# mmbajo/PROBA-V

Hardware: AMD Instinct MI355X
Metric: LR-patches/sec fwd+bwd (WDSR-B r12 t9, 16x16, bs128) (higher is better)
Workload: dtype f32 (products as 3 scaled-fp16-piece MFMA products, f32 accumulate)

## Files before the change

include/probav_hip.h:

```cpp
#ifndef PROBAV_HIP_H
#define PROBAV_HIP_H
#include <stddef.h>
#include <stdint.h>
#ifdef __cplusplus
extern "C" {
#endif

#define PROBAV_ABI_VERSION 7

typedef struct probav_net_cfg {
    int32_t scale;
    int32_t num_filters;
    int32_t num_res_blocks;
    int32_t exp_rate;
    int32_t dec_channels;
    int32_t num_img_lr;
    int32_t patch_size_lr;
    int32_t max_shift;
    float mean, std;
    int32_t in_channels;
} probav_net_cfg;

typedef struct probav_engine probav_engine;

// ... 67 lines not shown
int probav_clip_round(const float* in, float* out, size_t n, float lo, float hi, void* stream);

int probav_conv3d_forward(const int32_t geom[17], const float* x, const float* gate, const float* w,
                          const float* bias, const float* skip, float* y, int impl, void* stream);
size_t probav_conv3d_wgrad_scratch_bytes(const int32_t geom[17], int impl);
int probav_conv3d_wgrad(const int32_t geom[17], const float* x, const float* dy, const float* gate,
                        float* dw, float* db, void* scratch, size_t scratch_bytes, int impl, void* stream);
int probav_pw_forward(const float* x, const float* w1, const float* b1, const float* w2, const float* b2, float* dec,
                      int64_t nvox, int64_t vox_per_sample, int D, int impl, void* stream);
size_t probav_pw_backward_scratch_bytes(int D);
int probav_pw_backward(const float* x, const float* d_dec, const float* d_skip, const float* w1, const float* b1,
                       const float* w2, float* dx, float* dw1, float* db1, float* dw2, float* db2, void* scratch,
                       size_t scratch_bytes, int64_t nvox, int64_t vox_per_sample, int D, int impl, void* stream);
int probav_input_grad(int batch, int H, int T, int C, const float* g, const float* act0, const float* wmain, const float* d1,
                      const float* gate1 , const float* w1, float stdv, float* dx, void* stream);
int64_t probav_weff_count(const probav_engine* e);
int64_t probav_cout_total(const probav_engine* e);
int probav_wn_forward(probav_engine* e, const float* params, float* weff, float* weffT, float* inv_norm, void* stream);
int probav_wn_backward(probav_engine* e, const float* params, const float* dweff, const float* inv_norm,
                       float* grads, void* stream);

int probav_engine_side_stream(probav_engine* e, int mode);

int probav_mfma_probe(const void* seed, float* sink, int iters, int launches, void* stream);
int probav_mfma_probe_shape(const void* seed, float* sink, int iters, int launches, int shape, void* stream);

#define PROBAV_VIEW_ACT 0
#define PROBAV_VIEW_DEC 1
#define PROBAV_VIEW_RED 2
#define PROBAV_VIEW_RESID1 3
#define PROBAV_VIEW_INPUT 4
int probav_workspace_view(const probav_engine* e, int batch, int training, int kind, int index, int64_t* offset_floats, int64_t* count);
int probav_debug_hidden(probav_engine* e, const float* params, const void* ws , size_t ws_bytes, int batch, int block, float* hidden,
                        float* dec_scratch ,
                        const void* wcache , void* stream);
int probav_debug_hidden_from_forward_kernel(int on);

#define PROBAV_PLAN_NONE 0
#define PROBAV_PLAN_CW4 1
#define PROBAV_PLAN_PP 2
#define PROBAV_PLAN_PSTRIP 3
#define PROBAV_PLAN_STRIP 4
#define PROBAV_PLAN_ROWTILE 5
#define PROBAV_PLAN_DIRECT 6
#define PROBAV_PLAN_WG4 7
#define PROBAV_PLAN_WGRAD_X6 8
// ... 103 lines not shown
```

proba-v_amd/_lib.py:

```python
import ctypes
import os
from ctypes import POINTER, c_char, c_char_p, c_float, c_int, c_int32, c_int64, c_size_t, c_uint8, c_void_p

CSRC = os.path.join(os.path.dirname(os.path.abspath(__file__)), "csrc")
LIB_PATH = os.path.join(CSRC, "libprobav_hip.so")

PROBAV_OK, PROBAV_EINVAL, PROBAV_ENOSPACE, PROBAV_EHIP = 0, -1, -2, -3


class NetCfg(ctypes.Structure):
    _fields_ = [("scale", c_int32), ("num_filters", c_int32), ("num_res_blocks", c_int32), ("exp_rate", c_int32),
                ("dec_channels", c_int32), ("num_img_lr", c_int32), ("patch_size_lr", c_int32),
                ("max_shift", c_int32), ("mean", c_float), ("std", c_float), ("in_channels", c_int32)]


class GuardCtl(ctypes.Structure):
    _fields_ = [("scale", c_float), ("skip", ctypes.c_uint32), ("skipped_total", ctypes.c_uint32), ("norm", c_float)]


SIGNATURES = {
    "probav_abi_version": (c_int, []),
    "probav_last_error": (c_char_p, []),
    "probav_engine_create": (c_int, [POINTER(NetCfg), POINTER(c_void_p)]),
    "probav_engine_destroy": (None, [c_void_p]),
# ... 20 lines not shown
    "probav_clip_round": (c_int, [c_void_p, c_void_p, c_size_t, c_float, c_float, c_void_p]),
    "probav_nadam_step": (c_int, [c_void_p, c_void_p, c_void_p, c_void_p, c_int64, c_float, c_float, c_float, c_float,
                                  c_float, c_float, c_float, c_void_p]),
    "probav_grad_guard_scratch_bytes": (c_size_t, [c_int64]),
    "probav_grad_guard": (c_int, [c_void_p, c_int64, c_float, c_int, c_void_p, c_size_t, c_void_p, c_void_p]),
    "probav_nadam_step_guarded": (c_int, [c_void_p, c_void_p, c_void_p, c_void_p, c_void_p, c_int64, c_float, c_float, c_float, c_float,
                                          c_float, c_float, c_float, c_float, c_void_p, c_void_p]),
    "probav_optimizer_step_fused_guarded": (c_int, [c_void_p, c_void_p, c_void_p, c_void_p, c_void_p, c_float, c_float, c_float, c_float, c_float, c_float,
                                                    c_float, c_void_p, c_size_t, c_void_p, c_float, c_void_p, c_void_p]),
    "probav_conv3d_forward": (c_int, [POINTER(c_int32 * 17), c_void_p, c_void_p, c_void_p, c_void_p, c_void_p,
                                      c_void_p, c_int, c_void_p]),
    "probav_conv3d_wgrad_scratch_bytes": (c_size_t, [POINTER(c_int32 * 17), c_int]),
    "probav_conv3d_wgrad": (c_int, [POINTER(c_int32 * 17), c_void_p, c_void_p, c_void_p, c_void_p, c_void_p,
                                    c_void_p, c_size_t, c_int, c_void_p]),
    "probav_pw_forward": (c_int, [c_void_p, c_void_p, c_void_p, c_void_p, c_void_p, c_void_p, c_int64, c_int64, c_int, c_int, c_void_p]),
    "probav_pw_backward_scratch_bytes": (c_size_t, [c_int]),
    "probav_pw_backward": (c_int, [c_void_p] * 12 + [c_size_t, c_int64, c_int64, c_int, c_int, c_void_p]),
    "probav_weff_count": (c_int64, [c_void_p]),
    "probav_cout_total": (c_int64, [c_void_p]),
    "probav_wn_forward": (c_int, [c_void_p, c_void_p, c_void_p, c_void_p, c_void_p, c_void_p]),
    "probav_wn_backward": (c_int, [c_void_p, c_void_p, c_void_p, c_void_p, c_void_p, c_void_p]),
    "probav_workspace_view": (c_int, [c_void_p, c_int, c_int, c_int, c_int, POINTER(c_int64), POINTER(c_int64)]),
    "probav_engine_side_stream": (c_int, [c_void_p, c_int]),
    "probav_weight_cache_build": (c_int, [c_void_p, c_void_p, c_void_p, c_size_t, c_void_p]),
    "probav_mfma_probe": (c_int, [c_void_p, c_void_p, c_int, c_int, c_void_p]),
    "probav_mfma_probe_shape": (c_int, [c_void_p, c_void_p, c_int, c_int, c_int, c_void_p]),
    "probav_debug_hidden": (c_int, [c_void_p, c_void_p, c_void_p, c_size_t, c_int, c_int, c_void_p, c_void_p, c_void_p, c_void_p]),
    "probav_debug_hidden_from_forward_kernel": (c_int, [c_int]),
    "probav_plan_conv": (c_int, [POINTER(c_int32 * 17), c_int, c_int, c_int, c_int, POINTER(c_int32 * 8)]),
    "probav_plan_pw": (c_int, [c_int64, c_int64, c_int, c_int, c_int, POINTER(c_int32 * 8)]),
    "probav_engine_set_gemm_route": (c_int, [c_void_p, c_int]),
    "probav_engine_gemm_route": (c_int, [c_void_p]),
    "probav_gemm_conv3d_forward": (c_int, [POINTER(c_int32 * 17), c_void_p, c_void_p, c_void_p, c_void_p, c_void_p, c_void_p, c_void_p]),
    "probav_gemm_conv3d_wgrad_scratch_bytes": (c_size_t, [POINTER(c_int32 * 17)]),
    "probav_gemm_conv3d_wgrad": (c_int, [POINTER(c_int32 * 17), c_void_p, c_void_p, c_void_p, c_void_p, c_void_p, c_void_p, c_size_t, c_void_p]),
    "probav_plan_conv_gemm": (c_int, [POINTER(c_int32 * 17), c_int, c_int, c_int, c_int, POINTER(c_int32 * 8)]),
    "probav_engine_route_counts": (c_int, [c_void_p, c_int, POINTER(c_int32 * 4)]),
    "probav_engine_launched_counts": (c_int, [c_void_p, POINTER(c_int32 * 4), c_int]),
    "probav_engine_set_gemm_pair": (c_int, [c_void_p, c_int]),
    "probav_engine_gemm_pair": (c_int, [c_void_p]),
    "probav_engine_pair_kind": (c_int, [c_void_p]),
    "probav_plan_pw_gemm": (c_int, [c_int, c_int, c_int, c_int64, c_int, POINTER(c_int32 * 8)]),
    "probav_engine_set_gemm_x6": (c_int, [c_void_p, c_int]),
    "probav_engine_gemm_x6": (c_int, [c_void_p]),
    "probav_engine_gemm_arith": (c_int, [c_void_p]),
    "probav_plan_conv_gemm_x6": (c_int, [POINTER(c_int32 * 17), c_int, c_int, c_int, POINTER(c_int32 * 8)]),
# ... 96 lines not shown
```

proba-v_amd/csrc/engine.hip:

```cpp
#include "probav_common.h"
#include "../../include/probav_hip.h"
#include <stdio.h>
#include <string.h>
#include <array>
#include <string>
#include <vector>

using namespace probav;

#include "kernels_mfma.h"
#include "kernels_x6.h"
#include "kernels_gemm.h"
#include "kernels_gemm_pw.h"
#include "kernels_gemm_x6.h"

struct ConvFrags { long f32 = -1, x6 = -1, h3 = -1, h3t = -1; };
struct PwFrags { long w1 = -1, w2 = -1, w2b = -1, w1c = -1; };

struct LayerRec {
    char name[32];
    WnLayer wn;
    int kh, kw, kt;
    ConvFrags pk[2];
};

enum class PairKind { none = 0, tuned = 1, gemm = 2 };
struct Family {
    bool mfma;
    bool strip;
    bool x6;
    int arith;
    PairKind pw_fused;
    bool gemm;
    int gemm_arith;
    bool gemm_exotic;
};
static Family make_family(int impl, bool pw_mfma, bool gemm = false, bool pair_gemm = false, bool gemm_x6 = false, bool gemm_exotic = false)
{
    Family f;
    f.mfma = impl >= 1; f.strip = impl >= 2; f.x6 = impl >= 3; f.arith = impl >= 4 ? 2 : (impl >= 3 ? 1 : 0);
    f.gemm = f.mfma && gemm;
    f.gemm_arith = f.gemm && gemm_x6 ? 1 : 0;
    f.gemm_exotic = f.gemm && gemm_exotic;
    f.pw_fused = !f.mfma ? PairKind::none : (pw_mfma ? PairKind::tuned : (f.gemm && pair_gemm ? PairKind::gemm : PairKind::none));
    return f;
}

struct probav_engine {
    probav_net_cfg cfg;
    std::vector<LayerRec> layers;
    int64_t nparams = 0, weff_count = 0, cout_total = 0, cin_total = 0;
    WnLayer* d_layers = nullptr;
    Family fam = {};
    int impl = 4;
    bool gemm = false;
    bool gemm_pair = false;
    bool gemm_x6 = false;
    bool gemm_exotic = false;
    bool pw_gemm = false;
    int32_t launched[4] = {0, 0, 0, 0};
    int iMain = -1, iResid1 = -1, iResid2 = -1, iResid3 = -1, iUp = -1;
    std::vector<int> iExp, iDec, iNorm, iRed;
    ReduceSide side = {};
    int side_mode = 2;
    bool side_tried = false;
    struct RedSpec { int k, p, pt, refl, refl_t; };
    std::vector<RedSpec> redSpec;
    int Hin = 0;
    std::vector<PackJob> jobs;
    PackJob* d_jobs = nullptr;
    int64_t wpack_count = 0;
    std::vector<std::array<PwFrags, 3>> pkBlk;
    bool pw_mfma = false;
    bool fwd_amax = false;
    PairKind fwd_pair = PairKind::none;
    int fwd_gemm_arith = 0;
    bool fwd_gemm_exotic = false;
    bool prof_on = false;
    unsigned prof_mask = ~0u;
    std::vector<hipEvent_t> prof_ev;
    std::vector<int> prof_cls;
    std::vector<double> prof_macs;
    size_t prof_used = 0;
};

static Family engine_family(const probav_engine* e) { return make_family(e->impl, e->pw_mfma, e->gemm, e->gemm_pair && e->pw_gemm, e->gemm_x6, e->gemm_exotic); }

enum { CLS_WN = 0, CLS_SMALL, CLS_CONV3_FWD, CLS_CONV3_BWD_DATA, CLS_CONV3_WGRAD, CLS_PW_FWD, CLS_PW_BWD_DATA, CLS_PW_WGRAD,
// ... 531 lines not shown
}
static int gemm_pair_backward_launch(const PassBufs& b, const Launch& L, const float* x, const float* dT, const float* dOut, float* dX, unsigned* ay, hipStream_t s)
{
    const probav_engine* e = b.e;
    const ConvGeom& g = L.g;
    const int i = L.i, D = e->cfg.dec_channels;
    if (L.kind != LaunchKind::fused || gemm_pw_backward_slab_floats(g.Cin, g.Cout, D, in_voxels(g)) > L.slab.floats) { set_error("probav_backward: the general fused pointwise pair's launch is not in the launch list, or its slab region is too small", hipSuccess); return PROBAV_EINVAL; }
    const WnLayer &we = e->layers[e->iExp[i]].wn, &wd = e->layers[e->iDec[i]].wn;
    CK(gemm_pw_backward(x, dT, dOut, b.dv.weff + we.w_off, b.params + we.b_off, b.dv.weff + wd.w_off, dX, b.dweff2 + we.w_off, b.dweff2 + wd.w_off,
                        b.grads + we.b_off, b.grads + wd.b_off, b.slabs + L.slab.off, in_voxels(g), g.Cin, g.Cout, D, s));
    if (ay) CK(amax_tensor(dX, (size_t)g.Hi * g.Wi * g.Ti * g.Cin, g.N, ay, s));
    return PROBAV_OK;
}

extern "C" {

int probav_abi_version(void) { return PROBAV_ABI_VERSION; }
int probav_engine_side_stream(probav_engine* e, int mode)
{
    if (!e || mode < 0 || mode > 2) { set_error("probav_engine_side_stream: bad argument", hipSuccess); return PROBAV_EINVAL; }
    e->side_mode = mode;
    return PROBAV_OK;
}
int probav_mfma_probe(const void* seed, float* sink, int iters, int launches, void* stream)
{
    if (!seed || !sink || iters < 1 || launches < 1) { set_error("probav_mfma_probe: null/invalid argument", hipSuccess); return PROBAV_EINVAL; }
    return mfma_probe(seed, sink, iters, launches, (hipStream_t)stream);
}
int probav_mfma_probe_shape(const void* seed, float* sink, int iters, int launches, int shape, void* stream)
{
    if (!seed || !sink || iters < 1 || launches < 1 || shape < 0 || shape > 1) { set_error("probav_mfma_probe_shape: null/invalid argument", hipSuccess); return PROBAV_EINVAL; }
    return mfma_probe(seed, sink, iters, launches, (hipStream_t)stream, shape);
}
const char* probav_last_error(void) { return probav::last_error(); }

int probav_engine_create(const probav_net_cfg* cfg, probav_engine** out)
{
    if (!cfg || !out) { set_error("probav_engine_create: null argument", hipSuccess); return PROBAV_EINVAL; }
    const int T = cfg->num_img_lr;
    if (cfg->scale != 3 || cfg->max_shift != 2 * cfg->scale) {
        set_error("probav_engine_create: the reference graph only closes for scale=3, maxShift=6 (models/modelsTF.py:45-53)", hipSuccess);
        return PROBAV_EINVAL;
    }
    if (T != 7 && T != 9 && T != 13 && T != 19) {
        set_error("probav_engine_create: numImgLR must be 7, 9, 13 or 19 (models/modelsTF.py:62-69)", hipSuccess);
        return PROBAV_EINVAL;
// ... 460 lines not shown
    CK(reduce_flush(s));
    for (int i = R - 1; i >= 0; --i) {
        float* gDec = S + p.gDec;
        float* Hbuf = S + p.Hb;
        float* dH = S + p.dH;
        const Launch pair = launch_at(p, Role::pair, LaunchKind::fused, true, i), dn = data(Role::norm, i);
        const bool fusedp = pair.kind == LaunchKind::fused;
        { Amax m; if (h3) { m.x = A.dec(i); m.w = acur; }
          CK(conv_wgrad(pb, filter(Role::norm, i), W + p.dec[i], cur, nullptr, m,
                        (fusedp && e->side_mode >= 2) ? (i < R - 1 ? reduce_fork_adjacent(s) : reduce_fork(s)) : s)); }
        if (fusedp) oth = S + p.gblk[i];
        unsigned* agdec = slot_of(dn);
        CK(conv_fwd(pb, dn, cur, nullptr, nullptr, gDec, amx(acur, e->iNorm[i], agdec), s));
        if (fusedp) {
            unsigned* anew = slot_of(pair);
            {
            const bool gp = e->fam.pw_fused == PairKind::gemm;
            ProfScope ps(e, (e->fam.x6 && !gp) ? CLS_PW_BWD_DATA_X6 : CLS_PW_BWD_DATA, (gp ? 3.0 : 2.0) * geom_macs(ge) + 2.0 * geom_macs(gd), s);
            if (gp) CK(gemm_pair_backward_launch(pb, pair, W + p.act[i], gDec, cur, oth, anew, s));
            else CK(pw_backward_launch(pb, pair, A, W + p.act[i], gDec, cur, oth, agdec, anew, s));
            }
            float* tmp2 = cur; cur = oth; oth = tmp2;
            acur = anew;
            if (((R - 1 - i) & 3) == 3 || i == 1) CK(reduce_flush(s));
            continue;
        }
        CK(conv_fwd(pb, data(Role::hidden, i), W + p.act[i], nullptr, nullptr, Hbuf, Amax(), s));
        CK(conv_wgrad(pb, filter(Role::dec, i), Hbuf, gDec, nullptr, Amax(), s));
        CK(conv_fwd(pb, data(Role::dec, i), gDec, nullptr, nullptr, dH, Amax(), s));
        CK(conv_wgrad(pb, filter(Role::exp, i), W + p.act[i], dH, Hbuf, Amax(), s));
        const Launch de = data(Role::exp, i);
        unsigned* aoth = slot_of(de);
        CK(conv_fwd(pb, de, dH, Hbuf, cur, oth, amx(nullptr, e->iExp[i], aoth), s));
        float* tmp = cur; cur = oth; oth = tmp;
        acur = aoth;
    }
    CK(reduce_flush(s));
    {
        ReduceSide* const ctx = side_guard.c;
        reduce_side_activate(nullptr);
        const int rc = conv_wgrad(pb, filter(Role::main), W + p.xn, cur, W + p.act[0], Amax(), s);
        reduce_side_activate(ctx);
        if (rc) return rc;
    }
    CK(reduce_join(s));
    if (dx) {
        CK(input_grad(B, e->Hin, e->cfg.num_img_lr, e->cfg.in_channels, cur, W + p.act[0], weff(e->iMain), S + p.dr1,
// ... 629 lines not shown
```

proba-v_amd/csrc/kernels_mfma.h:

```cpp
#pragma once
#include "probav_common.h"
#include "w4_switch.h"

namespace probav {

enum { PACK_CONV = 0, PACK_PW_A_KCIN = 1, PACK_PW_A_KHCH = 2, PACK_PW_A_KOUT = 3, PACK_PW_A_CIN_KHCH = 4,
       PACK_X6_PW_W1 = 10, PACK_X6_PW_W2 = 11, PACK_X6_CONV = 12, PACK_X6_PW_W2K = 13, PACK_X6_PW_W1C = 14, PACK_X6_CONVK = 15, PACK_X6_CONVP = 16,
       PACK_H3_PW_W1 = 20, PACK_H3_PW_W2 = 21, PACK_H3_CONV = 22, PACK_H3_PW_W2K = 23, PACK_H3_PW_W1C = 24, PACK_H3_CONVK = 25,
       PACK_H3_CONVP = 26 };
constexpr long X6_PW_FRAG_WORDS = 8 * 2 * 3 * 64 * 4;
constexpr long X6_CONV_FRAG_WORDS = 27 * 2 * 3 * 64 * 4;
constexpr long X6_CONVK_FRAG_WORDS = 9 * 5 * 3 * 64 * 4;
constexpr long H3_PW_FRAG_WORDS = 8 * 2 * 2 * 64 * 4;
constexpr long H3_CONV_FRAG_WORDS = 27 * 2 * 2 * 64 * 4;
constexpr long H3_CONVK_FRAG_WORDS = 9 * 5 * 2 * 64 * 4;

struct PackJob {
    int type, src_is_T;
    long src_off, dst_off, count;
    int Cin, Cout, CC, KS, taps;
    int amax_slot;
    int amax_percol, ncol;
};

// ... 13 lines not shown
    int nsplit, Wt;
    int nslot;
    unsigned mNslot;
};
struct StripPlan { bool ok; int CC, KS; size_t lds_bytes; int grid; StripArgs a; };
enum class StripKernel { none, cw4, pp, pstrip, strip };
struct StripSel { StripKernel k = StripKernel::none; int arith = 0, rvp = 2; bool taps = false; StripPlan plan = {}; };
StripSel strip_select(const ConvGeom& g, bool gated, int arith);
int conv_strip_forward(const StripSel& sel, const float* x, const float* gate, const float* wfrag, const float* bias,
                       const float* skip, float* y, const Amax& am, hipStream_t s);
bool x6_conv_rowtile_supported(const ConvGeom& g);
int x6_conv_rowtile_forward(const ConvGeom& g, const float* x, const float* gate, const float* wfrag6, const float* bias,
                            const float* skip, float* y, int arith, const Amax& am, hipStream_t s);
bool mfma_conv_plan_ints(const ConvGeom& g, bool wgrad, int out[3]);
bool mfma_wgrad_supported(const ConvGeom& g);
size_t mfma_wgrad_partial_floats(const ConvGeom& g);
int mfma_conv_wgrad(const ConvGeom& g, const float* x, const float* dy, const float* gate, float* dw, float* db,
                    float* partial, hipStream_t s);

bool mfma_pw_supported(int F, int E, int D);
int mfma_pw_forward(const float* x, const float* w1frag, const float* w2frag, const float* b1, const float* b2, float* dec,
                    long nvox, int D, hipStream_t s);

size_t mfma_pw_backward_slab_floats(int D);
int mfma_pw_backward(const float* x, const float* dT, const float* dOut, const float* w1kcin, const float* w2kout,
                     const float* w1khch, const float* b1, float* dX, float* dW1, float* dW2, float* db1, float* db2,
                     float* slabs, long nvox, int D, hipStream_t s);

int mfma_wgrad_reduce(const float* partial, const float* partial_b, float* dw, float* db, long nw, int Cout, int slabs, hipStream_t s);
int mfma_pw_backward_reduce(const float* slabs, int D, float* dW1, float* dW2, float* db1, float* db2, hipStream_t s);
int mfma_pw_backward_grid();

bool cw4_conv_supported(const ConvGeom& g, bool gated);
bool cw4_conv_plan_ints(const ConvGeom& g, bool gated, int out[5]);
int cw4_conv_forward(const ConvGeom& g, const float* x, const float* wfrag, const float* bias, const float* skip, float* y, const Amax& am, hipStream_t s);

}
```

proba-v_amd/csrc/kernels_mfma.hip:

```cpp
#include "probav_common.h"
#include "kernels_mfma.h"
#include "x6_device.h"
#include <type_traits>
#include <cstdint>


namespace probav {

#if defined(PROBAV_STAMP_CLOCK) && !defined(PROBAV_STAMP)
__device__ unsigned long long g_stamps[8192 * 8];
#endif
#ifdef PROBAV_STAMP
__device__ unsigned long long g_stamps[8192 * 8];
#define STAMP(k) do { if (threadIdx.x == 0 && blockIdx.x < 8192) g_stamps[blockIdx.x * 8 + (k)] = __builtin_amdgcn_s_memtime(); } while (0)
#define STAMP_DECL unsigned long long st_t0 = 0, st_fill = 0, st_steps = 0
#define STAMP_T0 st_t0 = __builtin_amdgcn_s_memtime()
#define STAMP_ACC(var) do { const unsigned long long t_ = __builtin_amdgcn_s_memtime(); var += t_ - st_t0; st_t0 = t_; } while (0)
#define STAMP_OUT do { if (threadIdx.x == 0 && blockIdx.x < 8192) { g_stamps[blockIdx.x * 8 + 1] = st_fill; g_stamps[blockIdx.x * 8 + 2] = st_steps; } } while (0)
#else
#define STAMP(k) do { } while (0)
#define STAMP_DECL do { } while (0)
#define STAMP_T0 do { } while (0)
#define STAMP_ACC(var) do { } while (0)
#define STAMP_OUT do { } while (0)
// ... 2589 lines not shown
            for (int s = 0; s < 16; ++s) { t1 += tr[s]; dW1 = MFMA32(xa[s], tr[s], dW1); }
            bs1 += t1;
        }
#pragma unroll
        for (int s = 0; s < 16; ++s) dW2 = MFMA32(tr2[s], dtb[s], dW2);
        __builtin_amdgcn_sched_barrier(0);
        asm volatile("" ::: "memory");
#pragma unroll
        for (int r = 0; r < 16; ++r) Tb[col * 33 + rowmap(r, half)] = dx[r];
        if (tnext < ntiles) stage_store(buf ^ 1, nxv, nd0, nd1);
        __syncthreads();
        {
            float s0 = do0, s1 = do1;
#pragma unroll
            for (int j = 0; j < PW2_WAVES; ++j) {
                const float* P = TbAll + j * 2 * PW2_TB;
                s0 += P[rv0 * 33 + col];
                s1 += P[rv1 * 33 + col];
            }
            if (rok0) dX[(v0 + rv0) * 32 + col] = s0;
            if (rok1) dX[(v0 + rv1) * 32 + col] = s1;
        }
    }
    const long slab_floats = 8192 + 256 * (long)D + 256 + D;
    float* sl = slabs + (long)blockIdx.x * slab_floats;
#pragma unroll
    for (int r = 0; r < 16; ++r) {
        const int rw = rowmap(r, half);
        sl[(long)rw * 256 + 32 * c + col] = dW1[r];
        if (col < D) sl[8192 + (long)(32 * c + rw) * D + col] = dW2[r];
    }
    const float b = bs1 + __shfl_xor(bs1, 32, 64);
    if (half == 0) sl[8192 + 256 * (long)D + 32 * c + col] = b;
    if (c == 0) {
        const float b2s = bs2 + __shfl_xor(bs2, 32, 64);
        if (half == 0 && col < D) sl[8192 + 256 * (long)D + 256 + col] = b2s;
    }
}

static const int PW_BWD_GRID = 256;

int mfma_pw_backward_reduce(const float* slabs, int D, float* dW1, float* dW2, float* db1, float* db2, hipStream_t s)
{
    const long slab_floats = 8192 + 256 * (long)D + 256 + D;
    SlabSumJob jobs[4] = {{slabs, dW1, slab_floats, 8192, PW_BWD_GRID}, {slabs + 8192, dW2, slab_floats, 256 * D, PW_BWD_GRID},
                          {slabs + 8192 + 256 * (long)D, db1, slab_floats, 256, PW_BWD_GRID}, {slabs + 8192 + 256 * (long)D + 256, db2, slab_floats, D, PW_BWD_GRID}};
    return slab_sum_later(s, jobs, 4);
}
int mfma_pw_backward_grid() { return PW_BWD_GRID; }

size_t mfma_pw_backward_slab_floats(int D) { return (size_t)PW_BWD_GRID * (8192 + 256 * (size_t)D + 256 + D); }

int mfma_pw_backward(const float* x, const float* dT, const float* dOut, const float* w1kcin, const float* w2kout,
                     const float* w1khch, const float* b1, float* dX, float* dW1, float* dW2, float* db1, float* db2,
                     float* slabs, long nvox, int D, hipStream_t s)
{
    const size_t lds = (size_t)(2 * PW2_XT + 2 * PW2_DT + PW2_WAVES * 2 * PW2_TB) * sizeof(float);
    const long slab_floats = 8192 + 256 * (long)D + 256 + D;
    const int rc = launch_lds<pw_bwd2_mfma_kernel>("pw_bwd2_mfma", dim3(PW_BWD_GRID), dim3(64 * PW2_WAVES), lds, s, x, dT, dOut, (const float4*)w1kcin,
                                                   (const float4*)w2kout, (const float4*)w1khch, b1, dX, slabs, nvox, D);
    if (rc) return rc;
    return mfma_pw_backward_reduce(slabs, D, dW1, dW2, db1, db2, s);
}

}
```

proba-v_amd/csrc/kernels_pw4.hip:

```cpp
#include "kernels_x6.h"
#include "x6_device.h"
#include <cstdlib>
#include <type_traits>

namespace probav {
#ifdef PW4_DIAG
namespace diag {
#endif
#ifdef PW4_STAMP
__device__ unsigned long long g_pw4_stamps[1024 * 16];
#define PW4_ST(k) do { unsigned long long t_; asm volatile("s_memtime %0\n\ts_waitcnt lgkmcnt(0)" : "=s"(t_) :: "memory"); st_acc[k] += t_ - st_prev; st_prev = t_; } while (0)
#else
#define PW4_ST(k) do { } while (0)
#endif

#ifdef PW4_ABL_NOMFMA
#define PW4_MFMA_V(a, b, c) (c)
#else
#define PW4_MFMA_V(a, b, c) __builtin_amdgcn_mfma_f32_32x32x16_f16((a).h, (b).h, (c), 0, 0, 0)
#endif
#ifdef PW4_ABL_NOMFMA
#define PW4_MFMA_A(acc, a, b) asm volatile("" : "+a"(acc) : "v"((a).h), "v"((b).h))
#define PW4_MFMA_AS(acc, a, b) asm volatile("" : "+a"(acc) : "v"((a).h), "v"((b).h))
#else
// ... 538 lines not shown
#pragma unroll
        for (int k = 0; k < 4; ++k) load_x(k);
#pragma unroll
        for (int k = 0; k < 16; ++k) load_d(k);
        boundary(std::true_type(), tb - 1);
        for (int t = tb; t < te; ++t) {
            iter(std::integral_constant<int, 0>(), std::false_type(), std::true_type(), t);
            iter(std::integral_constant<int, 1>(), std::true_type(), std::true_type(), t);
            iter(std::integral_constant<int, 2>(), std::true_type(), std::true_type(), t);
            iter(std::integral_constant<int, 3>(), std::true_type(), std::true_type(), t);
            iter(std::integral_constant<int, 4>(), std::true_type(), std::true_type(), t);
            iter(std::integral_constant<int, 5>(), std::true_type(), std::true_type(), t);
            iter(std::integral_constant<int, 6>(), std::true_type(), std::true_type(), t);
            iter(std::integral_constant<int, 7>(), std::true_type(), std::false_type(), t);
            boundary(std::false_type(), t);
        }
        if (am.y) amax_commit(omax, am.y + n);
    }
#ifdef PW4_STAMP
    st_acc[8] = __builtin_amdgcn_s_memtime() - st_c0; st_acc[9] = __builtin_amdgcn_s_memrealtime() - st_r0;
    if (lane == 0 && gw < 1024) { for (int k = 0; k < 10; ++k) g_pw4_stamps[gw * 16 + k] = st_acc[k]; g_pw4_stamps[gw * 16 + 10] = st_r0 - st_entry; g_pw4_stamps[gw * 16 + 11] = __builtin_amdgcn_s_memrealtime(); }
#endif

    const long slab_floats = 8192 + 256 * (long)D + 256 + D;
    float* sl = slabs + (long)blockIdx.x * slab_floats;
    const int lane2 = (int)__builtin_amdgcn_mbcnt_hi(~0u, __builtin_amdgcn_mbcnt_lo(~0u, 0u)), tid2 = wave * 64 + lane2;
    float* R = reinterpret_cast<float*>(lds);
    __syncthreads();
#ifdef PW4_STAMP
    if (lane2 == 0 && gw < 1024) g_pw4_stamps[gw * 16 + 12] = __builtin_amdgcn_s_memrealtime();
#endif
#pragma unroll
    for (int c = 0; c < 8; ++c)
#pragma unroll
        for (int r = 0; r < 16; ++r) R[((wave * 8 + c) * 16 + r) * 64 + lane2] = ldexpf(dW1[c][r], -(ex + eg));
    __syncthreads();
    for (int e4 = tid2; e4 < 2048; e4 += 256) {
        const float4 a = reinterpret_cast<const float4*>(R)[e4], b = reinterpret_cast<const float4*>(R + 8192)[e4],
                     c4 = reinterpret_cast<const float4*>(R + 2 * 8192)[e4], d = reinterpret_cast<const float4*>(R + 3 * 8192)[e4];
        const int e = 4 * e4, l = e & 63, r = (e >> 6) & 15, c = e >> 10;
        float* o = sl + (long)rowmap(r, l >> 5) * 256 + 32 * c + (l & 31);
        o[0] = ((a.x + b.x) + c4.x) + d.x; o[1] = ((a.y + b.y) + c4.y) + d.y; o[2] = ((a.z + b.z) + c4.z) + d.z; o[3] = ((a.w + b.w) + c4.w) + d.w;
    }
    __syncthreads();
#pragma unroll
    for (int c = 0; c < 8; ++c)
#pragma unroll
        for (int r = 0; r < 16; ++r) R[((wave * 8 + c) * 16 + r) * 64 + lane2] = ldexpf(dW2t[c][r], -(ed + eh));
    float* R1 = R + 4 * 8192;
#pragma unroll
    for (int c = 0; c < 8; ++c) R1[(wave * 8 + c) * 64 + lane2] = ldexpf(bs1[c], -eg);
    R1[4 * 8 * 64 + wave * 64 + lane2] = ldexpf(bs2, -ed);
    __syncthreads();
    for (int o = tid2; o < 256 * D; o += 256) {
        const int hid = o / D, out = o - hid * D;
        const int e = (((hid >> 5) * 16 + (out & 3) + 4 * (out >> 3)) * 64) + (hid & 31) + 32 * ((out >> 2) & 1);
        sl[8192 + o] = ((R[e] + R[8192 + e]) + R[2 * 8192 + e]) + R[3 * 8192 + e];
    }
    {
        const int c = tid2 >> 5, hcol = tid2 & 31;
        float v = 0.f;
#pragma unroll
        for (int w = 0; w < 4; ++w) v += R1[(w * 8 + c) * 64 + hcol] + R1[(w * 8 + c) * 64 + 32 + hcol];
        sl[8192 + 256 * (long)D + tid2] = v;
        if (tid2 < D) {
            float u = 0.f;
#pragma unroll
            for (int w = 0; w < 4; ++w) u += R1[4 * 8 * 64 + w * 64 + tid2] + R1[4 * 8 * 64 + w * 64 + 32 + tid2];
            sl[8192 + 256 * (long)D + 256 + tid2] = u;
        }
    }
#ifdef PW4_STAMP
    if (lane2 == 0 && gw < 1024) g_pw4_stamps[gw * 16 + 13] = __builtin_amdgcn_s_memrealtime();
#endif
}

bool pw4_backward_supported(long nvox, long vps, int D)
{
    if (vps <= 0 || nvox % vps || D != 25) return false;
    const long nsamp = nvox / vps;
    return nsamp >= 1 && nsamp <= 4L * mfma_pw_backward_grid() && vps < (1L << 26);
}

int pw4_backward_wps(long nvox, long vps) { return (int)(4L * mfma_pw_backward_grid() / (nvox / vps)); }

int pw4_backward(const float* x, const float* dT, const float* dOut, const float* w1f, const float* w2kf, const float* w1cf,
                 const float* b1, float* dX, float* dW1, float* dW2, float* db1, float* db2, float* slabs, long nvox, long vps, int D,
                 const PwAmax& am, hipStream_t s)
{
    if (!pw4_backward_supported(nvox, vps, D)) { set_error("pw4_backward: unsupported shape", hipSuccess); return PROBAV_EINVAL; }
    if (!am.x || !am.w1 || !am.w2 || !am.b1 || !am.dt || !am.w1r) { set_error("pw4_backward: H3 arithmetic needs the operands' amax slots", hipSuccess); return PROBAV_EINVAL; }
    const int grid = mfma_pw_backward_grid(), nsamp = (int)(nvox / vps);
    const int wps = pw4_backward_wps(nvox, vps);
// ... 11 lines not shown
```

proba-v_amd/csrc/kernels_x6.hip:

```cpp
#include "kernels_x6.h"
#include "x6_device.h"
#include <type_traits>
#include <cstdlib>


namespace probav {


#ifdef PROBAV_STAMP
#define PF_ACC(k) do { __builtin_amdgcn_sched_barrier(0); XS_ACC(k); __builtin_amdgcn_sched_barrier(0); } while (0)
#else
#define PF_ACC(k) do { } while (0)
#endif
template <class AR> struct PwfShape { static constexpr int WAVES = 12, WGS = 1; };
template <> struct PwfShape<H3> { static constexpr int WAVES = 8, WGS = 2; };

template <class AR, bool DUMP>
__global__ __launch_bounds__(64 * PwfShape<AR>::WAVES, PwfShape<AR>::WGS) void pw_fwd_x6_kernel(const float* __restrict__ x, const uint4* __restrict__ w1frag,
                                                                     const uint4* __restrict__ w2frag, const float* __restrict__ b1,
                                                                     const float* __restrict__ b2, float* __restrict__ dec,
                                                                     long nvox, int vps, int D, PwAmax am, float* __restrict__ hdump)
{
    constexpr int NP = AR::NP, PWF_WAVES = PwfShape<AR>::WAVES;
    extern __shared__ __attribute__((aligned(16))) unsigned char lds_raw[];
// ... 449 lines not shown
        const int nrem = vps - 32 * sj < 32 ? vps - 32 * sj : 32;
        {
            const bool xl = (tid >> 3) < nrem;
            unsigned a[NP], b[NP];
            cut_pair<AR>(xl ? xv.x : 0.f, xl ? xv.y : 0.f, sx, a);
            cut_pair<AR>(xl ? xv.z : 0.f, xl ? xv.w : 0.f, sx, b);
            unsigned char* dst = XA + buf * PB_TILE + (tid >> 3) * PB_ROW + (tid & 7) * 8;
#pragma unroll
            for (int p = 0; p < NP; ++p) *reinterpret_cast<uint2*>(dst + p * PB_IMG) = make_uint2(a[p], b[p]);
        }
#pragma unroll
        for (int k = 0; k < 4; ++k) {
            const float dv = tid + 256 * k < nrem * D ? d[k] : 0.f;
            if (tid + 256 * k < 32 * D) {
                unsigned short q[NP];
                cut_one<AR>(dv, sd, q);
                unsigned char* dst = DA + buf * PB_TILE + dvk[k] * PB_ROW + dok[k] * 2;
#pragma unroll
                for (int p = 0; p < NP; ++p) *reinterpret_cast<unsigned short*>(dst + p * PB_IMG) = q[p];
            }
            bs2[k] += dv;
        }
    };
    const long slab_floats = 8192 + 256 * (long)D + 256 + D;
    float* sl = slabs + (long)blockIdx.x * slab_floats;
    bool flushed = false;
    auto flush = [&](const Sc& q) {
        asm volatile("" ::: "memory");
        float a1[16], a2[16], a3[16];
#pragma unroll
        for (int r = 0; r < 16; ++r) {
            a1[r] = dW1[r]; a2[r] = dW2t[r];
            if constexpr (AR::SCALED) { a1[r] = ldexpf(a1[r], -(q.ex + q.eg)); a2[r] = ldexpf(a2[r], -(q.ed + q.eh)); }
            float v = bs1v[r];
#pragma unroll
            for (int m = 1; m < 32; m <<= 1) v += __shfl_xor(v, m, 64);
            if constexpr (AR::SCALED) v = ldexpf(v, -q.eg);
            a3[r] = v;
            dW1[r] = 0.f; dW2t[r] = 0.f; bs1v[r] = 0.f;
        }
        if (flushed) {
#pragma unroll
            for (int r = 0; r < 16; ++r) {
                const int rw = rowmap(r, half);
                a1[r] += sl[(long)rw * 256 + 32 * c + col];
                if (rw < D) a2[r] += sl[8192 + (long)(32 * c + col) * D + rw];
                if (col == 0) a3[r] += sl[8192 + 256 * (long)D + 32 * c + rw];
            }
        }
#pragma unroll
        for (int r = 0; r < 16; ++r) {
            const int rw = rowmap(r, half);
            sl[(long)rw * 256 + 32 * c + col] = a1[r];
            if (rw < D) sl[8192 + (long)(32 * c + col) * D + rw] = a2[r];
            if (col == 0) sl[8192 + 256 * (long)D + 32 * c + rw] = a3[r];
        }
        flushed = true;
    };

    int tile = tbeg;
    int n = tbeg / tps, j = tbeg - n * tps;
    int buf = 0;
    XS_DECL;
#ifdef PROBAV_STAMP2
    unsigned long long xs2[8] = {0, 0, 0, 0, 0, 0, 0, 0}, xs2t = 0;
#endif
    __syncthreads();
    if (tile < tend) cur = sample_scales(n);
    if (tid < 256) sB1[tid] = b1[tid] * pow2i(cur.eh);
    if (tile < tend) {
        float4 xv = make_float4(0.f, 0.f, 0.f, 0.f); float d[4] = {0.f, 0.f, 0.f, 0.f};
        stage_load(n, j, xv, d);
        stage_store(0, j, xv, d, pow2i(cur.ex), pow2i(cur.ed));
    }
    const int rk0 = wave < 4 ? 0 : 2;
    long pv0 = -1; int pnrem = 0, pn = -1, pkdx = 0;
    float pdo[4] = {0.f, 0.f, 0.f, 0.f};
    auto reduce_prev = [&](int pb) {
// ... 182 lines not shown
    };
    while (tile < tend) {
        int seg_last = (n + 1) * tps - 1;
        if (seg_last > tend - 1) seg_last = tend - 1;
        for (; tile < seg_last; ++tile, buf ^= 1) do_tile(std::false_type());
        do_tile(std::true_type());
        ++tile; buf ^= 1;
    }
    __syncthreads();
    reduce_prev(buf ^ 1);
    commit_done();
    if (am.y && pn >= 0) amax_commit(omax, am.y + pn);
    flush(cur);
    __syncthreads();
    float* R = TbAll;
    if (stager) {
#pragma unroll
        for (int k = 0; k < 4; ++k) R[tid + 256 * k] = (tid + 256 * k < 32 * D) ? bs2[k] : 0.f;
    }
    __syncthreads();
    if (tid < D) {
        float t = 0.f;
        for (int jj = tid; jj < 1024; jj += D) t += R[jj];
        sl[8192 + 256 * (long)D + 256 + tid] = t;
    }
    XS_ACC(6);
    XS_OUT;
#ifdef PROBAV_STAMP2
    if ((threadIdx.x & 63) == 0 && blockIdx.x < 1024) for (int k_ = 0; k_ < 5; ++k_) g_stamps[(blockIdx.x * 8 + (threadIdx.x >> 6)) * 8 + 1 + k_] = xs2[k_];
#endif
}


enum class PwBwdKernel { w4, x6_h3, x6 };
static PwBwdKernel x6_pw_backward_select(long nvox, long vps, int D, int arith)
{
    if (arith != 2) return PwBwdKernel::x6;
    return w4_enabled(W4::pw_bwd) && pw4_backward_supported(nvox, vps, D) ? PwBwdKernel::w4 : PwBwdKernel::x6_h3;
}

int x6_pw_backward(const float* x, const float* dT, const float* dOut, const float* w1f, const float* w2kf, const float* w1cf,
                   const float* b1, float* dX, float* dW1, float* dW2, float* db1, float* db2, float* slabs, long nvox, long vps, int D,
                   int arith, const PwAmax& am, hipStream_t s)
{
    if (vps <= 0 || vps > nvox) vps = nvox;
    if (nvox % vps || vps > 0x7fffffffL) { set_error("x6_pw_backward: nvox must be a multiple of the voxels per sample", hipSuccess); return PROBAV_EINVAL; }
    if (arith == 2 && (!am.x || !am.w1 || !am.w2 || !am.b1 || !am.dt || !am.w1r)) { set_error("x6_pw_backward: H3 arithmetic needs the operands' amax slots", hipSuccess); return PROBAV_EINVAL; }
// ... 545 lines not shown
```

proba-v_amd/modelsTF.py:

```python
import contextlib
import ctypes
import os
import weakref
from ctypes import c_char, c_int32, c_int64, c_void_p, byref

import torch

from . import _lib, ops
from .arch import layer_table


class WDSRModel(torch.nn.Module):

    def __init__(self, name, band, mean, std, maxShift, scale, numFilters, numResBlocks, expRate, decayRate,
                 numImgLR, patchSizeLR, seed=None, inChannels=1):
        super().__init__()
        self.name, self.band = name, band
        self.mean, self.std, self.maxShift = float(mean), float(std), int(maxShift)
        self.scale, self.numFilters, self.numResBlocks = int(scale), int(numFilters), int(numResBlocks)
        self.expRate, self.decayRate = int(expRate), float(decayRate)
        self.numImgLR, self.patchSizeLR = int(numImgLR), int(patchSizeLR)
        self.inChannels = int(inChannels)
        self.arch = dict(numFilters=self.numFilters, numResBlocks=self.numResBlocks, expRate=self.expRate,
                         decayRate=self.decayRate, numImgLR=self.numImgLR, scale=self.scale, inChannels=self.inChannels)
# ... 149 lines not shown
    @property
    def gemm_pair(self):
        return bool(_lib.lib().probav_engine_gemm_pair(self._handle()))

    def set_gemm_x6(self, on):
        _lib.check(_lib.lib().probav_engine_set_gemm_x6(self._handle(), int(bool(on))), "probav_engine_set_gemm_x6")
        ops.forget_engine(self._handle().value)

    @property
    def gemm_x6(self):
        return bool(_lib.lib().probav_engine_gemm_x6(self._handle()))

    def set_gemm_exotic(self, on):
        _lib.check(_lib.lib().probav_engine_set_gemm_exotic(self._handle(), int(bool(on))), "probav_engine_set_gemm_exotic")
        ops.forget_engine(self._handle().value)

    @property
    def gemm_exotic(self):
        return bool(_lib.lib().probav_engine_gemm_exotic(self._handle()))

    def set_side_stream_mode(self, mode):
        _lib.check(_lib.lib().probav_engine_side_stream(self._handle(), int(mode)), "probav_engine_side_stream")

    def tune_side_stream(self, step, steps=8, rounds=2, modes=(2, 1)):
        import statistics
        ms = {m: [] for m in modes}
        for _ in range(rounds):
            for m in modes:
                self.set_side_stream_mode(m)
                step()
                a, b = torch.cuda.Event(enable_timing=True), torch.cuda.Event(enable_timing=True)
                torch.cuda.synchronize()
                a.record()
                for _ in range(steps):
                    step()
                b.record()
                torch.cuda.synchronize()
                ms[m].append(a.elapsed_time(b) / steps)
        med = {m: statistics.median(v) for m, v in ms.items()}
        best = min(med, key=med.get)
        self.set_side_stream_mode(best)
        return best, med

    def weight_cache_buffer(self):
        if self._wcache is None or self._wcache.device != self.flat.device:
            n = _lib.lib().probav_weight_cache_bytes(self._handle())
# ... 176 lines not shown
```

Before: 21040.

## Split pointwise-backward slabs into per-field regions and vectorize the pw4 epilogue stores

The per-workgroup gradient slab layout changes from interleaved records (dW1, dW2, db1, db2 per block) to separate contiguous regions per field. This lets the slab-sum reduction read each field with a dense stride. The pw4 backward epilogue now stores dW1 as float4 when aligned. It also transposes dW2 through LDS so that dW2 goes out with coalesced float4 writes, and it keeps only the 13 row blocks needed. A runtime knob for the reduce-flush cadence is added, with the default unchanged at 4. The risks are the extra LDS staging, an additional barrier, and a possible layout mismatch with any other consumer of the slab buffer.

```diff
diff --git a/include/probav_hip.h b/include/probav_hip.h
--- a/include/probav_hip.h
+++ b/include/probav_hip.h
@@ -113,6 +113,8 @@
 
 int probav_engine_side_stream(probav_engine* e, int mode);
 
+int probav_engine_set_slab_flush_blocks(probav_engine* e, int blocks);
+
 int probav_mfma_probe(const void* seed, float* sink, int iters, int launches, void* stream);
 int probav_mfma_probe_shape(const void* seed, float* sink, int iters, int launches, int shape, void* stream);
 
diff --git a/proba-v_amd/_lib.py b/proba-v_amd/_lib.py
--- a/proba-v_amd/_lib.py
+++ b/proba-v_amd/_lib.py
@@ -66,6 +66,7 @@
     "probav_wn_backward": (c_int, [c_void_p, c_void_p, c_void_p, c_void_p, c_void_p, c_void_p]),
     "probav_workspace_view": (c_int, [c_void_p, c_int, c_int, c_int, c_int, POINTER(c_int64), POINTER(c_int64)]),
     "probav_engine_side_stream": (c_int, [c_void_p, c_int]),
+    "probav_engine_set_slab_flush_blocks": (c_int, [c_void_p, c_int]),
     "probav_weight_cache_build": (c_int, [c_void_p, c_void_p, c_void_p, c_size_t, c_void_p]),
     "probav_mfma_probe": (c_int, [c_void_p, c_void_p, c_int, c_int, c_void_p]),
     "probav_mfma_probe_shape": (c_int, [c_void_p, c_void_p, c_int, c_int, c_int, c_void_p]),
diff --git a/proba-v_amd/csrc/engine.hip b/proba-v_amd/csrc/engine.hip
--- a/proba-v_amd/csrc/engine.hip
+++ b/proba-v_amd/csrc/engine.hip
@@ -45,6 +45,8 @@
     f.pw_fused = !f.mfma ? PairKind::none : (pw_mfma ? PairKind::tuned : (f.gemm && pair_gemm ? PairKind::gemm : PairKind::none));
     return f;
 }
+
+constexpr int SLAB_FLUSH_BLOCKS = 4;
 
 struct probav_engine {
     probav_net_cfg cfg;
@@ -64,6 +66,7 @@
     ReduceSide side = {};
     int side_mode = 2;
     bool side_tried = false;
+    int slab_flush_blocks = SLAB_FLUSH_BLOCKS;
     struct RedSpec { int k, p, pt, refl, refl_t; };
     std::vector<RedSpec> redSpec;
     int Hin = 0;
@@ -641,6 +644,12 @@
     e->side_mode = mode;
     return PROBAV_OK;
 }
+int probav_engine_set_slab_flush_blocks(probav_engine* e, int blocks)
+{
+    if (!e || blocks < 1) { set_error("probav_engine_set_slab_flush_blocks: bad argument", hipSuccess); return PROBAV_EINVAL; }
+    e->slab_flush_blocks = blocks;
+    return PROBAV_OK;
+}
 int probav_mfma_probe(const void* seed, float* sink, int iters, int launches, void* stream)
 {
     if (!seed || !sink || iters < 1 || launches < 1) { set_error("probav_mfma_probe: null/invalid argument", hipSuccess); return PROBAV_EINVAL; }
@@ -1147,7 +1156,7 @@
             }
             float* tmp2 = cur; cur = oth; oth = tmp2;
             acur = anew;
-            if (((R - 1 - i) & 3) == 3 || i == 1) CK(reduce_flush(s));
+            if ((R - 1 - i) % e->slab_flush_blocks == e->slab_flush_blocks - 1 || i == 1) CK(reduce_flush(s));
             continue;
         }
         CK(conv_fwd(pb, data(Role::hidden, i), W + p.act[i], nullptr, nullptr, Hbuf, Amax(), s));
diff --git a/proba-v_amd/csrc/kernels_mfma.h b/proba-v_amd/csrc/kernels_mfma.h
--- a/proba-v_amd/csrc/kernels_mfma.h
+++ b/proba-v_amd/csrc/kernels_mfma.h
@@ -59,6 +59,13 @@
 int mfma_pw_forward(const float* x, const float* w1frag, const float* w2frag, const float* b1, const float* b2, float* dec,
                     long nvox, int D, hipStream_t s);
 
+constexpr int PW_BWD_SLABS = 256;
+struct PwSlab { float *dW1, *dW2, *db1, *db2; };
+__host__ __device__ inline PwSlab pw_backward_slab(float* region, int D, int wg)
+{
+    float* const s2 = region + (long)PW_BWD_SLABS * 8192, * const s3 = s2 + (long)PW_BWD_SLABS * 256 * D, * const s4 = s3 + (long)PW_BWD_SLABS * 256;
+    return {region + (long)wg * 8192, s2 + (long)wg * 256 * D, s3 + (long)wg * 256, s4 + (long)wg * D};
+}
 size_t mfma_pw_backward_slab_floats(int D);
 int mfma_pw_backward(const float* x, const float* dT, const float* dOut, const float* w1kcin, const float* w2kout,
                      const float* w1khch, const float* b1, float* dX, float* dW1, float* dW2, float* db1, float* db2,
diff --git a/proba-v_amd/csrc/kernels_mfma.hip b/proba-v_amd/csrc/kernels_mfma.hip
--- a/proba-v_amd/csrc/kernels_mfma.hip
+++ b/proba-v_amd/csrc/kernels_mfma.hip
@@ -2635,29 +2635,27 @@
             if (rok1) dX[(v0 + rv1) * 32 + col] = s1;
         }
     }
-    const long slab_floats = 8192 + 256 * (long)D + 256 + D;
-    float* sl = slabs + (long)blockIdx.x * slab_floats;
+    const PwSlab sl = pw_backward_slab(slabs, D, blockIdx.x);
 #pragma unroll
     for (int r = 0; r < 16; ++r) {
         const int rw = rowmap(r, half);
-        sl[(long)rw * 256 + 32 * c + col] = dW1[r];
-        if (col < D) sl[8192 + (long)(32 * c + rw) * D + col] = dW2[r];
+        sl.dW1[(long)rw * 256 + 32 * c + col] = dW1[r];
+        if (col < D) sl.dW2[(long)(32 * c + rw) * D + col] = dW2[r];
     }
     const float b = bs1 + __shfl_xor(bs1, 32, 64);
-    if (half == 0) sl[8192 + 256 * (long)D + 32 * c + col] = b;
+    if (half == 0) sl.db1[32 * c + col] = b;
     if (c == 0) {
         const float b2s = bs2 + __shfl_xor(bs2, 32, 64);
-        if (half == 0 && col < D) sl[8192 + 256 * (long)D + 256 + col] = b2s;
-    }
-}
-
-static const int PW_BWD_GRID = 256;
+        if (half == 0 && col < D) sl.db2[col] = b2s;
+    }
+}
+
+static const int PW_BWD_GRID = PW_BWD_SLABS;
 
 int mfma_pw_backward_reduce(const float* slabs, int D, float* dW1, float* dW2, float* db1, float* db2, hipStream_t s)
 {
-    const long slab_floats = 8192 + 256 * (long)D + 256 + D;
-    SlabSumJob jobs[4] = {{slabs, dW1, slab_floats, 8192, PW_BWD_GRID}, {slabs + 8192, dW2, slab_floats, 256 * D, PW_BWD_GRID},
-                          {slabs + 8192 + 256 * (long)D, db1, slab_floats, 256, PW_BWD_GRID}, {slabs + 8192 + 256 * (long)D + 256, db2, slab_floats, D, PW_BWD_GRID}};
+    const PwSlab f = pw_backward_slab(const_cast<float*>(slabs), D, 0);
+    SlabSumJob jobs[4] = {{f.dW1, dW1, 8192, 8192, PW_BWD_GRID}, {f.dW2, dW2, 256 * (long)D, 256 * D, PW_BWD_GRID}, {f.db1, db1, 256, 256, PW_BWD_GRID}, {f.db2, db2, (long)D, D, PW_BWD_GRID}};
     return slab_sum_later(s, jobs, 4);
 }
 int mfma_pw_backward_grid() { return PW_BWD_GRID; }
@@ -2669,7 +2667,6 @@
                      float* slabs, long nvox, int D, hipStream_t s)
 {
     const size_t lds = (size_t)(2 * PW2_XT + 2 * PW2_DT + PW2_WAVES * 2 * PW2_TB) * sizeof(float);
-    const long slab_floats = 8192 + 256 * (long)D + 256 + D;
     const int rc = launch_lds<pw_bwd2_mfma_kernel>("pw_bwd2_mfma", dim3(PW_BWD_GRID), dim3(64 * PW2_WAVES), lds, s, x, dT, dOut, (const float4*)w1kcin,
                                                    (const float4*)w2kout, (const float4*)w1khch, b1, dX, slabs, nvox, D);
     if (rc) return rc;
diff --git a/proba-v_amd/csrc/kernels_pw4.hip b/proba-v_amd/csrc/kernels_pw4.hip
--- a/proba-v_amd/csrc/kernels_pw4.hip
+++ b/proba-v_amd/csrc/kernels_pw4.hip
@@ -584,8 +584,8 @@
     if (lane == 0 && gw < 1024) { for (int k = 0; k < 10; ++k) g_pw4_stamps[gw * 16 + k] = st_acc[k]; g_pw4_stamps[gw * 16 + 10] = st_r0 - st_entry; g_pw4_stamps[gw * 16 + 11] = __builtin_amdgcn_s_memrealtime(); }
 #endif
 
-    const long slab_floats = 8192 + 256 * (long)D + 256 + D;
-    float* sl = slabs + (long)blockIdx.x * slab_floats;
+    const PwSlab sl = pw_backward_slab(slabs, D, blockIdx.x);
+    const bool al16 = (reinterpret_cast<unsigned long long>(slabs) & 15ull) == 0ull;
     const int lane2 = (int)__builtin_amdgcn_mbcnt_hi(~0u, __builtin_amdgcn_mbcnt_lo(~0u, 0u)), tid2 = wave * 64 + lane2;
     float* R = reinterpret_cast<float*>(lds);
     __syncthreads();
@@ -601,36 +601,53 @@
         const float4 a = reinterpret_cast<const float4*>(R)[e4], b = reinterpret_cast<const float4*>(R + 8192)[e4],
                      c4 = reinterpret_cast<const float4*>(R + 2 * 8192)[e4], d = reinterpret_cast<const float4*>(R + 3 * 8192)[e4];
         const int e = 4 * e4, l = e & 63, r = (e >> 6) & 15, c = e >> 10;
-        float* o = sl + (long)rowmap(r, l >> 5) * 256 + 32 * c + (l & 31);
-        o[0] = ((a.x + b.x) + c4.x) + d.x; o[1] = ((a.y + b.y) + c4.y) + d.y; o[2] = ((a.z + b.z) + c4.z) + d.z; o[3] = ((a.w + b.w) + c4.w) + d.w;
+        float* o = sl.dW1 + (long)rowmap(r, l >> 5) * 256 + 32 * c + (l & 31);
+        const float4 v = make_float4(((a.x + b.x) + c4.x) + d.x, ((a.y + b.y) + c4.y) + d.y, ((a.z + b.z) + c4.z) + d.z, ((a.w + b.w) + c4.w) + d.w);
+        if (al16) *reinterpret_cast<float4*>(o) = v;
+        else { o[0] = v.x; o[1] = v.y; o[2] = v.z; o[3] = v.w; }
     }
     __syncthreads();
+    constexpr int NRB = 13, WB = 8 * NRB * 64;
+    float* R1 = R + 4 * WB;
+    float* T = R1 + (4 * 8 + 4) * 64;
+    static_assert((4 * WB + (4 * 8 + 4) * 64 + 256 * 25) * (int)sizeof(float) <= PW4_LDS, "the epilogue's images must fit the launch's LDS");
 #pragma unroll
     for (int c = 0; c < 8; ++c)
 #pragma unroll
-        for (int r = 0; r < 16; ++r) R[((wave * 8 + c) * 16 + r) * 64 + lane2] = ldexpf(dW2t[c][r], -(ed + eh));
-    float* R1 = R + 4 * 8192;
+        for (int r = 0; r < NRB; ++r) R[((wave * 8 + c) * NRB + r) * 64 + lane2] = ldexpf(dW2t[c][r], -(ed + eh));
 #pragma unroll
     for (int c = 0; c < 8; ++c) R1[(wave * 8 + c) * 64 + lane2] = ldexpf(bs1[c], -eg);
     R1[4 * 8 * 64 + wave * 64 + lane2] = ldexpf(bs2, -ed);
     __syncthreads();
-    for (int o = tid2; o < 256 * D; o += 256) {
-        const int hid = o / D, out = o - hid * D;
-        const int e = (((hid >> 5) * 16 + (out & 3) + 4 * (out >> 3)) * 64) + (hid & 31) + 32 * ((out >> 2) & 1);
-        sl[8192 + o] = ((R[e] + R[8192 + e]) + R[2 * 8192 + e]) + R[3 * 8192 + e];
+    for (int e4 = tid2; e4 < WB / 4; e4 += 256) {
+        const float4 a = reinterpret_cast<const float4*>(R)[e4], b = reinterpret_cast<const float4*>(R + WB)[e4],
+                     c4 = reinterpret_cast<const float4*>(R + 2 * WB)[e4], d = reinterpret_cast<const float4*>(R + 3 * WB)[e4];
+        const int e = 4 * e4, l = e & 63, cr = e >> 6, c = cr / NRB, r = cr - c * NRB;
+        const int out = rowmap(r, l >> 5);
+        if (out < D) {
+            float* t = T + (32 * c + (l & 31)) * D + out;
+            t[0] = ((a.x + b.x) + c4.x) + d.x; t[D] = ((a.y + b.y) + c4.y) + d.y; t[2 * D] = ((a.z + b.z) + c4.z) + d.z; t[3 * D] = ((a.w + b.w) + c4.w) + d.w;
+        }
     }
     {
         const int c = tid2 >> 5, hcol = tid2 & 31;
         float v = 0.f;
 #pragma unroll
         for (int w = 0; w < 4; ++w) v += R1[(w * 8 + c) * 64 + hcol] + R1[(w * 8 + c) * 64 + 32 + hcol];
-        sl[8192 + 256 * (long)D + tid2] = v;
+        sl.db1[tid2] = v;
         if (tid2 < D) {
             float u = 0.f;
 #pragma unroll
             for (int w = 0; w < 4; ++w) u += R1[4 * 8 * 64 + w * 64 + tid2] + R1[4 * 8 * 64 + w * 64 + 32 + tid2];
-            sl[8192 + 256 * (long)D + 256 + tid2] = u;
+            sl.db2[tid2] = u;
         }
+    }
+    __syncthreads();
+    for (int q = tid2; q < 64 * D; q += 256) {
+        const float4 v = reinterpret_cast<const float4*>(T)[q];
+        float* o = sl.dW2 + 4 * q;
+        if (al16) *reinterpret_cast<float4*>(o) = v;
+        else { o[0] = v.x; o[1] = v.y; o[2] = v.z; o[3] = v.w; }
     }
 #ifdef PW4_STAMP
     if (lane2 == 0 && gw < 1024) g_pw4_stamps[gw * 16 + 13] = __builtin_amdgcn_s_memrealtime();
diff --git a/proba-v_amd/csrc/kernels_x6.hip b/proba-v_amd/csrc/kernels_x6.hip
--- a/proba-v_amd/csrc/kernels_x6.hip
+++ b/proba-v_amd/csrc/kernels_x6.hip
@@ -495,8 +495,7 @@
             bs2[k] += dv;
         }
     };
-    const long slab_floats = 8192 + 256 * (long)D + 256 + D;
-    float* sl = slabs + (long)blockIdx.x * slab_floats;
+    const PwSlab sl = pw_backward_slab(slabs, D, blockIdx.x);
     bool flushed = false;
     auto flush = [&](const Sc& q) {
         asm volatile("" ::: "memory");
@@ -516,17 +515,17 @@
 #pragma unroll
             for (int r = 0; r < 16; ++r) {
                 const int rw = rowmap(r, half);
-                a1[r] += sl[(long)rw * 256 + 32 * c + col];
-                if (rw < D) a2[r] += sl[8192 + (long)(32 * c + col) * D + rw];
-                if (col == 0) a3[r] += sl[8192 + 256 * (long)D + 32 * c + rw];
+                a1[r] += sl.dW1[(long)rw * 256 + 32 * c + col];
+                if (rw < D) a2[r] += sl.dW2[(long)(32 * c + col) * D + rw];
+                if (col == 0) a3[r] += sl.db1[32 * c + rw];
             }
         }
 #pragma unroll
         for (int r = 0; r < 16; ++r) {
             const int rw = rowmap(r, half);
-            sl[(long)rw * 256 + 32 * c + col] = a1[r];
-            if (rw < D) sl[8192 + (long)(32 * c + col) * D + rw] = a2[r];
-            if (col == 0) sl[8192 + 256 * (long)D + 32 * c + rw] = a3[r];
+            sl.dW1[(long)rw * 256 + 32 * c + col] = a1[r];
+            if (rw < D) sl.dW2[(long)(32 * c + col) * D + rw] = a2[r];
+            if (col == 0) sl.db1[32 * c + rw] = a3[r];
         }
         flushed = true;
     };
@@ -755,7 +754,7 @@
     if (tid < D) {
         float t = 0.f;
         for (int jj = tid; jj < 1024; jj += D) t += R[jj];
-        sl[8192 + 256 * (long)D + 256 + tid] = t;
+        sl.db2[tid] = t;
     }
     XS_ACC(6);
     XS_OUT;
diff --git a/proba-v_amd/modelsTF.py b/proba-v_amd/modelsTF.py
--- a/proba-v_amd/modelsTF.py
+++ b/proba-v_amd/modelsTF.py
@@ -195,6 +195,9 @@
     def set_side_stream_mode(self, mode):
         _lib.check(_lib.lib().probav_engine_side_stream(self._handle(), int(mode)), "probav_engine_side_stream")
 
+    def set_slab_flush_blocks(self, blocks):
+        _lib.check(_lib.lib().probav_engine_set_slab_flush_blocks(self._handle(), int(blocks)), "probav_engine_set_slab_flush_blocks")
+
     def tune_side_stream(self, step, steps=8, rounds=2, modes=(2, 1)):
         import statistics
         ms = {m: [] for m in modes}
```

New measurement: 21180 (median of 6 runs). No clear change (+0.6%).
